# fjarri-attic/pyfft

Measured on AMD Instinct MI355X. Metric: batched_c2c_fft_gflops_5NlogN_1d_n2^20, higher is better.
Workload: dtype f32

## Files before the change

include/mifft.h:

```cpp
#ifndef MIFFT_H
#define MIFFT_H

#include <stddef.h>
#include <stdint.h>

#ifdef __cplusplus
extern "C" {
#endif

#define MIFFT_ABI_VERSION 6

#define MIFFT_E_INVALID      (-1)
#define MIFFT_E_UNSUPPORTED  (-2)
#define MIFFT_E_NODEVICE     (-3)

#define MIFFT_F32 0
#define MIFFT_F64 1

#define MIFFT_INTERLEAVED 0
#define MIFFT_SPLIT       1

#define MIFFT_FLAG_SRC_INTERLEAVED 1
#define MIFFT_FLAG_DST_INTERLEAVED 2
#define MIFFT_FLAG_STREAM_SRC 4
// ... 27 lines not shown
    int32_t tw_shift;
    int32_t src;
    int32_t dst;
    int32_t flags;
} mifft_pass;

typedef struct mifft_device_props {
    char    name[256];
    char    gcn_arch[64];
    int32_t compute_units;
    int32_t wavefront_size;
    int32_t max_threads_per_block;
    int32_t max_grid_x;
    int64_t lds_bytes_per_block;
    int64_t total_mem_bytes;
    int32_t clock_khz;
    int32_t l2_bytes;
    int64_t llc_bytes;
    int32_t num_xcc;
    int32_t reserved0;
} mifft_device_props;

int         mifft_abi_version(void);
const char *mifft_last_error(void);
#define MIFFT_DEBUG_NO_ND2 0
#define MIFFT_DEBUG_NO_WAVE 2
#define MIFFT_DEBUG_FORCE_WAVE 3
#define MIFFT_DEBUG_ALT_ROWS 5
#define MIFFT_DEBUG_PAIR 6
#define MIFFT_DEBUG_STORE 7
#define MIFFT_DEBUG_ROWS_ND 8
#define MIFFT_DEBUG_NARROW_TILES 9
#define MIFFT_DEBUG_NO_ROWFIRST 10
#define MIFFT_DEBUG_KEYS 12
int mifft_debug_set(int32_t key, int32_t value);
int mifft_debug_set_default(int32_t key, int32_t value);
int mifft_debug_get(int32_t key);

int mifft_device_count(int *count);
int mifft_set_device(int device);
int mifft_get_device(int *device);
int mifft_device_props_get(int device, mifft_device_props *props);
int mifft_malloc(void **ptr, size_t nbytes);
int mifft_free(void *ptr);
int mifft_memset(void *ptr, int value, size_t nbytes, mifft_stream_t stream);
int mifft_memcpy_h2d(void *dst, const void *src, size_t nbytes, mifft_stream_t stream);
int mifft_memcpy_d2h(void *dst, const void *src, size_t nbytes, mifft_stream_t stream);
int mifft_memcpy_d2d(void *dst, const void *src, size_t nbytes, mifft_stream_t stream);
int mifft_host_alloc(void **ptr, size_t nbytes);
int mifft_host_free(void *ptr);
int mifft_memcpy_d2h_async(void *dst, const void *src, size_t nbytes, mifft_stream_t stream);
int mifft_stream_create(mifft_stream_t *stream);
int mifft_stream_destroy(mifft_stream_t stream);
int mifft_stream_sync(mifft_stream_t stream);
int mifft_device_sync(void);
typedef void *mifft_graph_t;
int mifft_stream_is_capturing(mifft_stream_t stream, int32_t *capturing);
int mifft_stream_begin_capture(mifft_stream_t stream);
int mifft_stream_end_capture(mifft_stream_t stream, mifft_graph_t *graph);
int mifft_graph_launch(mifft_graph_t graph, mifft_stream_t stream);
int mifft_graph_destroy(mifft_graph_t graph);
int mifft_event_create(mifft_event_t *event);
int mifft_event_destroy(mifft_event_t event);
int mifft_event_record(mifft_event_t event, mifft_stream_t stream);
int mifft_event_sync(mifft_event_t event);
int mifft_event_query(mifft_event_t event);
int mifft_stream_wait_event(mifft_stream_t stream, mifft_event_t event);
int mifft_event_elapsed_ms(float *ms, mifft_event_t start, mifft_event_t stop);


// ... 163 lines not shown
```

pyfft_amd/_debug.py:

```python
import os


def forced_strategy():
    return os.environ.get("PYFFT_AMD_STRATEGY", "auto")


def pipeline_chunk_bytes(default):
    return (int(os.environ.get("PYFFT_AMD_PIPE_MB", "0")) << 20) or default


def no_nd_generic():
    return bool(os.environ.get("PYFFT_AMD_NO_ND_GENERIC"))


def pipeline_streams(default):
    return int(os.environ.get("PYFFT_AMD_PIPE_STREAMS", "0")) or default


def slab_bytes(default):
    return (int(os.environ.get("PYFFT_AMD_SLAB_MB", "0")) << 20) or default


def no_slabs():
    return bool(os.environ.get("PYFFT_AMD_NO_SLABS"))
# ... 40 lines not shown

def no_fusedp_alt():
    return bool(os.environ.get("PYFFT_AMD_NO_FUSEDP_ALT"))


def no_tiled_kernel():
    return bool(os.environ.get("PYFFT_AMD_NO_TILED"))


def no_mixed_nd():
    return bool(os.environ.get("PYFFT_AMD_NO_MIXED_ND"))


def fused3_lag_ring(lag, ring):
    v = os.environ.get("PYFFT_AMD_FUSED3")
    if v:
        lag, ring = (int(t) for t in v.split(","))
    return lag, ring


def apply_native_switches(native):
    for env, key in (("MIFFT_NO_ND2", native.DEBUG_NO_ND2), ("MIFFT_NO_WAVE", native.DEBUG_NO_WAVE),
                     ("MIFFT_FORCE_WAVE", native.DEBUG_FORCE_WAVE)):
        if os.environ.get(env):
            native.lib.mifft_debug_set_default(key, 1)
    if os.environ.get("MIFFT_STORE"):
        native.lib.mifft_debug_set_default(native.DEBUG_STORE, int(os.environ["MIFFT_STORE"]))
    if os.environ.get("MIFFT_ROWS_ND"):
        native.lib.mifft_debug_set_default(native.DEBUG_ROWS_ND, int(os.environ["MIFFT_ROWS_ND"]))
    if os.environ.get("MIFFT_NARROW_TILES"):
        native.lib.mifft_debug_set_default(native.DEBUG_NARROW_TILES, int(os.environ["MIFFT_NARROW_TILES"]))
    if os.environ.get("MIFFT_PAIR"):
        native.lib.mifft_debug_set_default(native.DEBUG_PAIR, int(os.environ["MIFFT_PAIR"]))
    if os.environ.get("PYFFT_AMD_NO_SPLIT_ROWFIRST"):
        native.lib.mifft_debug_set_default(native.DEBUG_NO_ROWFIRST, 1)
```

pyfft_amd/_native.py:

```python

import ctypes
import os

_HERE = os.path.dirname(os.path.abspath(__file__))
LIB_PATH = os.path.join(_HERE, "libmifft.so")

ABI_VERSION = 6
MIFFT_MIXED_MAX_STAGES = 12

E_INVALID = -1
E_UNSUPPORTED = -2
E_NODEVICE = -3

F32, F64 = 0, 1
INTERLEAVED, SPLIT = 0, 1
VARIANT_INTERLEAVED_ONLY = 2
VARIANT_SPLIT_ONLY = 3
VARIANT_OUT_OF_PLACE_ONLY = 4
VARIANT_OUT_OF_PLACE_ANY_SIZE = 5
VARIANT_SPLIT_OUT_OF_PLACE = 6
VARIANT_SPLIT_OUT_OF_PLACE_ANY_SIZE = 7
PASS_COL, PASS_ROW, PASS_ND = 0, 1, 2
FLAG_SRC_INTERLEAVED, FLAG_DST_INTERLEAVED = 1, 2
FLAG_STREAM_SRC, FLAG_STREAM_DST = 4, 8
FLAG_WRITE_THROUGH = 32
FLAG_PAIR_WITH_NEXT = 16
HALF_KERNEL_TILE, HALF_KERNEL_ROW, HALF_KERNEL_ND2, HALF_KERNEL_ND = 1, 2, 3, 4
ND_KERNEL_WAVE, ND_KERNEL_ND2Z, ND_KERNEL_ND2, ND_KERNEL_ND2ZP, ND_KERNEL_ND2P, ND_KERNEL_ND2T, ND_KERNEL_ND = 1, 2, 3, 4, 5, 6, 7
FUSED2_COUNTER_STRIDE = 64


def fused2_counter_bytes(outer):
    return FUSED2_COUNTER_STRIDE * 4 * (9 + 2 * int(outer))


DEBUG_NO_ND2, DEBUG_NO_WAVE, DEBUG_FORCE_WAVE, DEBUG_ALT_ROWS, DEBUG_PAIR, DEBUG_STORE = 0, 2, 3, 5, 6, 7
DEBUG_ROWS_ND = 8
DEBUG_NARROW_TILES = 9
DEBUG_NO_ROWFIRST = 10
DEBUG_KEYS = 12


class MifftPass(ctypes.Structure):
    _fields_ = [
        ("kind", ctypes.c_int32),
        ("precision", ctypes.c_int32),
        ("layout", ctypes.c_int32),
        ("inverse", ctypes.c_int32),
        ("L", ctypes.c_int32),
        ("variant", ctypes.c_int32),
        ("M", ctypes.c_int64),
        ("S", ctypes.c_int64),
        ("outer", ctypes.c_int64),
        ("outer_stride_in", ctypes.c_int64),
        ("outer_stride_out", ctypes.c_int64),
        ("scale", ctypes.c_double),
        ("tw_L", ctypes.c_void_p),
        ("tw_lo", ctypes.c_void_p),
        ("tw_hi", ctypes.c_void_p),
        ("tw_shift", ctypes.c_int32),
        ("src", ctypes.c_int32),
        ("dst", ctypes.c_int32),
        ("flags", ctypes.c_int32),
    ]


class MifftCopy(ctypes.Structure):
    _fields_ = [
        ("precision", ctypes.c_int32),
        ("ndim", ctypes.c_int32),
        ("dims", ctypes.c_int64 * 6),
        ("src_stride", ctypes.c_int64 * 6),
        ("dst_stride", ctypes.c_int64 * 6),
# ... 62 lines not shown

class MifftRealPost(ctypes.Structure):
    _fields_ = [
        ("precision", ctypes.c_int32),
        ("inverse", ctypes.c_int32),
        ("nx", ctypes.c_int32),
        ("ny", ctypes.c_int32),
        ("nz", ctypes.c_int32),
        ("reserved", ctypes.c_int32),
        ("outer", ctypes.c_int64),
        ("stride_in", ctypes.c_int64),
        ("stride_out", ctypes.c_int64),
        ("in_", ctypes.c_void_p),
        ("out", ctypes.c_void_p),
        ("tw", ctypes.c_void_p),
        ("scale", ctypes.c_double),
    ]


_vp = ctypes.c_void_p
_vpp = ctypes.POINTER(ctypes.c_void_p)
_i32 = ctypes.c_int32
_sz = ctypes.c_size_t
_pass_p = ctypes.POINTER(MifftPass)
_sync_p = ctypes.POINTER(MifftFusedSync)
_buf3 = ctypes.c_void_p * 3

PROTOTYPES = {
    "mifft_abi_version": (ctypes.c_int, []),
    "mifft_last_error": (ctypes.c_char_p, []),
    "mifft_debug_set": (ctypes.c_int, [_i32, _i32]),
    "mifft_debug_set_default": (ctypes.c_int, [_i32, _i32]),
    "mifft_debug_get": (ctypes.c_int, [_i32]),
    "mifft_device_count": (ctypes.c_int, [ctypes.POINTER(ctypes.c_int)]),
    "mifft_set_device": (ctypes.c_int, [ctypes.c_int]),
    "mifft_get_device": (ctypes.c_int, [ctypes.POINTER(ctypes.c_int)]),
    "mifft_device_props_get": (ctypes.c_int, [ctypes.c_int, ctypes.POINTER(MifftDeviceProps)]),
    "mifft_malloc": (ctypes.c_int, [_vpp, _sz]),
    "mifft_free": (ctypes.c_int, [_vp]),
    "mifft_memset": (ctypes.c_int, [_vp, ctypes.c_int, _sz, _vp]),
    "mifft_memcpy_h2d": (ctypes.c_int, [_vp, _vp, _sz, _vp]),
    "mifft_memcpy_d2h": (ctypes.c_int, [_vp, _vp, _sz, _vp]),
    "mifft_memcpy_d2d": (ctypes.c_int, [_vp, _vp, _sz, _vp]),
    "mifft_host_alloc": (ctypes.c_int, [_vpp, _sz]),
    "mifft_host_free": (ctypes.c_int, [_vp]),
    "mifft_memcpy_d2h_async": (ctypes.c_int, [_vp, _vp, _sz, _vp]),
    "mifft_stream_create": (ctypes.c_int, [_vpp]),
    "mifft_stream_destroy": (ctypes.c_int, [_vp]),
    "mifft_stream_sync": (ctypes.c_int, [_vp]),
    "mifft_device_sync": (ctypes.c_int, []),
    "mifft_stream_is_capturing": (ctypes.c_int, [_vp, ctypes.POINTER(ctypes.c_int32)]),
    "mifft_stream_begin_capture": (ctypes.c_int, [_vp]),
    "mifft_stream_end_capture": (ctypes.c_int, [_vp, _vpp]),
    "mifft_graph_launch": (ctypes.c_int, [_vp, _vp]),
    "mifft_graph_destroy": (ctypes.c_int, [_vp]),
    "mifft_event_create": (ctypes.c_int, [_vpp]),
    "mifft_event_destroy": (ctypes.c_int, [_vp]),
    "mifft_event_record": (ctypes.c_int, [_vp, _vp]),
    "mifft_event_sync": (ctypes.c_int, [_vp]),
    "mifft_event_query": (ctypes.c_int, [_vp]),
    "mifft_stream_wait_event": (ctypes.c_int, [_vp, _vp]),
    "mifft_event_elapsed_ms": (ctypes.c_int, [ctypes.POINTER(ctypes.c_float), _vp, _vp]),
    "mifft_nd_max_points_for": (ctypes.c_int, [_i32]),
    "mifft_nd_shape_supported": (ctypes.c_int, [_i32, _i32, _i32, _i32, _i32]),
    "mifft_pass_supported": (ctypes.c_int, [_i32, _i32, _i32, _i32]),
    "mifft_launch_pass": (ctypes.c_int, [_pass_p, _vp, _vp, _vp, _vp, _vp]),
# ... 94 lines not shown
```

pyfft_amd/csrc/fft_col2.hpp:

```cpp
#pragma once
#include "fft_tile.hpp"

namespace mifft {

template <int A, int E, typename T> __device__ __forceinline__ cplx<T> mul_w16A(cplx<T> v) {
    if constexpr (A == 4)
        return mul_w64<E, T>(v);
    else
        return mul_w32<E, T>(v);
}

template <typename T> struct ColStageTw {
    cplx<T> s1, s2, s3, s4, s5, s6, s7, s8;
    __device__ __forceinline__ void init(const cplx<T>* twL, int i0, int step = 1) {
        load(twL, i0, step);
        finish();
    }
    __device__ __forceinline__ void load(const cplx<T>* twL, int i0, int step = 1) {
        s1 = twL[step * i0]; s2 = twL[2 * step * i0]; s4 = twL[4 * step * i0]; s8 = twL[8 * step * i0];
    }
    __device__ __forceinline__ void finish() {
        s3 = cmul<T>(s1, s2); s5 = cmul<T>(s4, s1); s6 = cmul<T>(s4, s2); s7 = cmul<T>(s4, s3);
    }
    template <int k> __device__ __forceinline__ cplx<T> get() const {
        if constexpr (k == 1) return s1;
        else if constexpr (k == 2) return s2;
        else if constexpr (k == 3) return s3;
        else if constexpr (k == 4) return s4;
        else if constexpr (k == 5) return s5;
        else if constexpr (k == 6) return s6;
        else if constexpr (k == 7) return s7;
        else if constexpr (k == 8) return s8;
        else if constexpr (k == 9) return cmul<T>(s8, s1);
        else if constexpr (k == 10) return cmul<T>(s8, s2);
        else if constexpr (k == 11) return cmul<T>(s8, s3);
        else if constexpr (k == 12) return cmul<T>(s8, s4);
        else if constexpr (k == 13) return cmul<T>(s8, s5);
        else if constexpr (k == 14) return cmul<T>(s8, s6);
        else return cmul<T>(s8, s7);
    }
};

template <int A, bool TR, int ESZ = 8> struct Col2Lds {
    static constexpr int PITCH = TR ? 17 : 16;
    static constexpr int BUF = 16 * 16 * PITCH;
    static constexpr bool DOUBLE = A > 2 && ESZ <= 8;
    static constexpr bool HALF = ESZ > 8;
    static constexpr int ELEMS = HALF ? (BUF + 1) / 2 : (DOUBLE ? 2 : 1) * BUF;
};

struct TileNoHook {
    __device__ __forceinline__ void operator()() const {}
};

template <typename T, int A, bool TR, bool TW, bool SPLIT, bool WT = false, bool NTIN = false, bool NTOUT = false,
          bool SPLIT_OUT = SPLIT, bool WIDE = false, typename LdsPtr = cplx<T>*, typename Hook = TileNoHook>
__device__ __forceinline__ void col2_tile(const TileArgs& a, const long long o_in, const long long o_out,
                                          const long long rem0, LdsPtr lds, Hook hook = Hook(), const int tid_in = -1) {
    constexpr int L = A * 256;
    constexpr int PPT = A * 16;
    constexpr int PITCH = Col2Lds<A, TR, sizeof(cplx<T>)>::PITCH;
    constexpr int BUF = Col2Lds<A, TR, sizeof(cplx<T>)>::BUF;
    constexpr bool kDoubleBuf = Col2Lds<A, TR, sizeof(cplx<T>)>::DOUBLE;
    constexpr bool kHalf = Col2Lds<A, TR, sizeof(cplx<T>)>::HALF;

    int tid = tid_in >= 0 ? tid_in : (int)threadIdx.x;
    asm volatile("" : "+v"(tid));
    const int cg = WIDE ? (tid & 31) : (tid & 15), b0 = WIDE ? (tid >> 5) : (tid >> 4);
    const int c = cg & 15;
    if constexpr (WIDE) lds = lds + (cg >> 4) * Col2Lds<A, TR, sizeof(cplx<T>)>::ELEMS;
    int logMS = a.logMS, logS = a.logS;
    asm volatile("" : "+s"(logMS), "+s"(logS));
    const cplx<T>* twL = reinterpret_cast<const cplx<T>*>(a.tw_L);
    const T csign = a.inverse ? (T)-1 : (T)1;

    cplx<T> v[PPT];
    {
        const long long ubase = o_in * a.ostride_in + rem0;
        const unsigned voff = (((unsigned)b0 << logMS) + (unsigned)cg);
        if constexpr (!SPLIT) {
            const char* src = reinterpret_cast<const char*>(reinterpret_cast<const cplx<T>*>(a.in0) + ubase);
            const unsigned vb = voff * (unsigned)sizeof(cplx<T>);
            static_for<PPT>([&](auto kk) {
                constexpr int k = kk, ia = k >> 4, b1 = k & 15;
                const char* p = src + (((long long)(b1 * 16 * A + ia * 16) << logMS) * (long long)sizeof(cplx<T>));
                if constexpr (NTIN)
                    v[k] = __builtin_nontemporal_load(reinterpret_cast<const cplx<T>*>(p + vb));
                else
                    v[k] = *reinterpret_cast<const cplx<T>*>(p + vb);
            });
        } else {
            const char* sre = reinterpret_cast<const char*>(reinterpret_cast<const T*>(a.in0) + ubase);
            const char* sim = reinterpret_cast<const char*>(reinterpret_cast<const T*>(a.in1) + ubase);
            const unsigned vb = voff * (unsigned)sizeof(T);
            static_for<PPT>([&](auto kk) {
                constexpr int k = kk, ia = k >> 4, b1 = k & 15;
                const long long off = ((long long)(b1 * 16 * A + ia * 16) << logMS) * (long long)sizeof(T);
                if constexpr (NTIN) {
                    v[k].x = __builtin_nontemporal_load(reinterpret_cast<const T*>(sre + off + vb));
                    v[k].y = __builtin_nontemporal_load(reinterpret_cast<const T*>(sim + off + vb));
                } else {
                    v[k].x = *reinterpret_cast<const T*>(sre + off + vb);
                    v[k].y = *reinterpret_cast<const T*>(sim + off + vb);
                }
            });
        }
    }
    const cplx<T> s1 = twL[b0], s2 = twL[2 * b0], s4 = twL[4 * b0], s8 = twL[8 * b0];
    cplx<T> twA[A > 1 ? A - 1 : 1];
    if constexpr (A > 1) {
        static_for<A - 1>([&](auto qq) {
            constexpr int qa = qq + 1;
            twA[qq] = twL[16 * b0 * qa];
        });
    }
    __builtin_amdgcn_sched_barrier(0);
    static_for<PPT>([&](auto kk) {
        constexpr int k = kk;
        v[k].y *= csign;
    });

    {
        const cplx<T> s3 = cmul<T>(s1, s2), s5 = cmul<T>(s4, s1), s6 = cmul<T>(s4, s2), s7 = cmul<T>(s4, s3);
        auto tw = [&](auto kk) -> cplx<T> {
            constexpr int k = kk;
            if constexpr (k == 1) return s1;
            else if constexpr (k == 2) return s2;
            else if constexpr (k == 3) return s3;
            else if constexpr (k == 4) return s4;
            else if constexpr (k == 5) return s5;
            else if constexpr (k == 6) return s6;
            else if constexpr (k == 7) return s7;
            else if constexpr (k == 8) return s8;
            else if constexpr (k == 9) return cmul<T>(s8, s1);
            else if constexpr (k == 10) return cmul<T>(s8, s2);
            else if constexpr (k == 11) return cmul<T>(s8, s3);
            else if constexpr (k == 12) return cmul<T>(s8, s4);
            else if constexpr (k == 13) return cmul<T>(s8, s5);
            else if constexpr (k == 14) return cmul<T>(s8, s6);
            else return cmul<T>(s8, s7);
        };
        static_for<A>([&](auto aa) {
            constexpr int ia = aa;
            Dft<16, T>::run(v + ia * 16);
            static_for<15>([&](auto q2) {
                constexpr int qb1 = q2 + 1;
                cplx<T> t = v[ia * 16 + qb1];
                if constexpr (ia > 0) t = mul_w16A<A, ia * qb1, T>(t);
                v[ia * 16 + qb1] = cmul<T>(t, tw(IC<qb1>{}));
            });
            __builtin_amdgcn_sched_barrier(0);
        });
    }
    if constexpr (A > 1) {
        static_for<16>([&](auto bb) {
            constexpr int qb1 = bb;
            cplx<T> t[A];
            static_for<A>([&](auto aa) {
                constexpr int ia = aa;
                t[ia] = v[ia * 16 + qb1];
            });
            Dft<A, T>::run(t);
            v[qb1] = t[0];
            static_for<A - 1>([&](auto qq) {
                constexpr int qa = qq + 1;
                v[qa * 16 + qb1] = cmul<T>(t[qa], twA[qq]);
            });
        });
    }
    __builtin_amdgcn_sched_barrier(0);
    hook();

    const int u = TR ? c : b0;
    const int c2 = TR ? b0 : c;
    const int c2g = WIDE ? ((cg & 16) + c2) : c2;
    const long long l0 = rem0 >> logS;
    const long long jp0 = rem0 & ((1ll << logS) - 1);
    const unsigned dl = (unsigned)(((rem0 + c2g) >> logS) - l0);
    const unsigned djp = (unsigned)(((rem0 + c2g) & ((1ll << logS) - 1)) - jp0);
    const unsigned l = (unsigned)l0 + dl;
    const T sx = (T)a.scale;
    const T sy = a.inverse ? -sx : sx;
    cplx<T> sxy;
    sxy.x = sx;
    sxy.y = sy;
    const cplx<T>* twlo = reinterpret_cast<const cplx<T>*>(a.tw_lo);
    const cplx<T>* twhi = reinterpret_cast<const cplx<T>*>(a.tw_hi);
    const int tw_shift = a.tw_shift;
    const unsigned lomask = (1u << tw_shift) - 1u;
    const long long oubase = TR ? (a.ostride_out * o_out + rem0 * L) : (a.ostride_out * o_out + ((l0 * L) << logS) + jp0);
    const unsigned ovoff = TR ? ((unsigned)c2g * L + (unsigned)u) : ((((unsigned)dl * L + (unsigned)u) << logS) + djp);

    cplx<T> nlo[TW ? 4 : 1], nhi[TW ? 4 : 1], sstep_lo, sstep_hi;
    auto look_ahead = [&](auto qq) {
        constexpr int qa = qq;
        if constexpr (TW) {
            static_for<4>([&](auto jj) {
                constexpr int j = jj;
                const unsigned e = l * (unsigned)(qa * 16 + u + 64 * A * j);
                nlo[j] = twlo[e & lomask];
                nhi[j] = twhi[e >> tw_shift];
            });
        }
    };
    if constexpr (TW) {
        const unsigned e = l * (16u * A);
        sstep_lo = twlo[e & lomask];
        sstep_hi = twhi[e >> tw_shift];
        look_ahead(IC<0>{});
        __builtin_amdgcn_sched_barrier(0);
    }

    static_for<A>([&](auto rr) {
        constexpr int qa = rr;
        LdsPtr buf = lds + (kDoubleBuf ? (qa & 1) * BUF : 0);
        if constexpr (!kDoubleBuf && qa > 0) __syncthreads();
        cplx<T> x[16];
        if constexpr (!kHalf) {
            static_for<16>([&](auto ss) {
                constexpr int qb1 = ss;
                if constexpr (TR)
                    buf[(b0 * 16 + c) * PITCH + qb1] = v[qa * 16 + qb1];
                else
                    buf[(b0 * 16 + qb1) * 16 + c] = v[qa * 16 + qb1];
// ... 24 lines not shown
                    constexpr int bi = bb;
                    T w;
                    if constexpr (TR)
                        w = sb[(bi * 16 + c2) * PITCH + u];
                    else
                        w = sb[(bi * 16 + u) * 16 + c2];
                    if constexpr (comp == 0) x[bi].x = w; else x[bi].y = w;
                });
            });
        }
        cplx<T> anchor[TW ? 4 : 1];
        cplx<T> sstep;
        if constexpr (TW) {
            static_for<4>([&](auto jj) { anchor[jj] = cmul<T>(nlo[jj], nhi[jj]); });
            sstep = cmul<T>(sstep_lo, sstep_hi);
            __builtin_amdgcn_sched_barrier(0);
            if constexpr (qa + 1 < A) {
                look_ahead(IC<qa + 1>{});
                __builtin_amdgcn_sched_barrier(0);
            }
        }
        Dft<16, T>::run(x);
        if constexpr (TW) {
            static_for<4>([&](auto jj) {
                constexpr int j = jj;
                cplx<T> cur = anchor[j];
                static_for<4>([&](auto ii) {
                    constexpr int qb0 = 4 * j + ii;
                    x[qb0] = cmul<T>(x[qb0], cur);
                    if constexpr (ii < 3) cur = cmul<T>(cur, sstep);
                });
            });
        }
        static_for<16>([&](auto qq) {
            constexpr int qb0 = qq;
            const long long gu = TR ? (oubase + qb0 * 16 * A + 16 * qa)
                                    : (oubase + ((long long)(qb0 * 16 * A + 16 * qa) << logS));
            const cplx<T> r = x[qb0] * sxy;
            if constexpr (!SPLIT_OUT) {
                char* p = reinterpret_cast<char*>(reinterpret_cast<cplx<T>*>(a.out0) + gu);
                if constexpr (WT) {
                    if constexpr (sizeof(cplx<T>) == 8)
                        __hip_atomic_store(reinterpret_cast<unsigned long long*>(p + ovoff * (unsigned)sizeof(cplx<T>)),
                                           __builtin_bit_cast(unsigned long long, r), __ATOMIC_RELAXED, __HIP_MEMORY_SCOPE_AGENT);
                    else
                        store_wt<T>(p, ovoff * (unsigned)sizeof(cplx<T>), r);
                } else if constexpr (NTOUT) {
                    __builtin_nontemporal_store(r, reinterpret_cast<cplx<T>*>(p + ovoff * (unsigned)sizeof(cplx<T>)));
                } else {
                    *reinterpret_cast<cplx<T>*>(p + ovoff * (unsigned)sizeof(cplx<T>)) = r;
                }
            } else {
                char* pr = reinterpret_cast<char*>(reinterpret_cast<T*>(a.out0) + gu);
                char* pi = reinterpret_cast<char*>(reinterpret_cast<T*>(a.out1) + gu);
                if constexpr (NTOUT) {
                    __builtin_nontemporal_store(r.x, reinterpret_cast<T*>(pr + ovoff * (unsigned)sizeof(T)));
                    __builtin_nontemporal_store(r.y, reinterpret_cast<T*>(pi + ovoff * (unsigned)sizeof(T)));
                } else {
                    *reinterpret_cast<T*>(pr + ovoff * (unsigned)sizeof(T)) = r.x;
                    *reinterpret_cast<T*>(pi + ovoff * (unsigned)sizeof(T)) = r.y;
                }
            }
        });
    });
}

template <typename T, int A, bool TR, bool TW, bool SPLIT, bool SPLIT_OUT = SPLIT>
__global__ void __launch_bounds__(256, 2) fft_col2_kernel(const TileArgs a) {
    __shared__ __attribute__((aligned(16))) cplx<T> lds[Col2Lds<A, TR, sizeof(cplx<T>)>::ELEMS];
    const long long col0 = (long long)blockIdx.x * 16;
    const long long o = col0 >> a.logMS;
    const long long rem0 = col0 & ((1ll << a.logMS) - 1);
    if constexpr (TR && !SPLIT) {
        if (a.nt & 4) col2_tile<T, A, TR, TW, SPLIT, true, false, false, SPLIT_OUT>(a, o, o, rem0, lds);
        else if (a.nt & 1) col2_tile<T, A, TR, TW, SPLIT, false, !SPLIT, false, SPLIT_OUT>(a, o, o, rem0, lds);
        else col2_tile<T, A, TR, TW, SPLIT, false, false, false, SPLIT_OUT>(a, o, o, rem0, lds);
    } else if constexpr (!TR && !SPLIT_OUT) {
        if (a.nt & 4) col2_tile<T, A, TR, TW, SPLIT, true, false, false, SPLIT_OUT>(a, o, o, rem0, lds);
        else if (a.nt & 2) col2_tile<T, A, TR, TW, SPLIT, false, false, !SPLIT_OUT, SPLIT_OUT>(a, o, o, rem0, lds);
        else col2_tile<T, A, TR, TW, SPLIT, false, false, false, SPLIT_OUT>(a, o, o, rem0, lds);
    } else {
        col2_tile<T, A, TR, TW, SPLIT, false, false, false, SPLIT_OUT>(a, o, o, rem0, lds);
    }
}

template <int A, bool TR, bool TW, bool SPLIT, bool SPLIT_OUT>
__global__ void __launch_bounds__(512, 2) fft_col2x_kernel(const TileArgs a) {
    using T = float;
    __shared__ __attribute__((aligned(16))) cplx<T> lds[2 * Col2Lds<A, TR, sizeof(cplx<T>)>::ELEMS];
    const long long col0 = (long long)blockIdx.x * 32;
    const long long o = col0 >> a.logMS;
    const long long rem0 = col0 & ((1ll << a.logMS) - 1);
    const int tid = threadIdx.x;
    if constexpr (TR) {
        if (a.nt & 4) col2_tile<T, A, TR, TW, SPLIT, true, false, false, SPLIT_OUT, true>(a, o, o, rem0, lds, TileNoHook(), tid);
        else if (a.nt & 1) col2_tile<T, A, TR, TW, SPLIT, false, true, false, SPLIT_OUT, true>(a, o, o, rem0, lds, TileNoHook(), tid);
// ... 9 lines not shown
```

pyfft_amd/csrc/fft_fused2.hpp:

```cpp
#pragma once
#include "fft_col2.hpp"
#include "fft_col2w.hpp"
#include "fft_col3.hpp"

namespace mifft {

constexpr unsigned kFusedCS = 64u;

struct FusedCtl {
    unsigned* counters;
    unsigned* counters_next;
    unsigned* err;
    unsigned lines;
    unsigned batch;
    unsigned lag;
    unsigned ring;
    unsigned tiles0;
    unsigned tiles1;
};

struct FusedArgs {
    TileArgs p0;
    TileArgs p1;
    FusedCtl c;
// ... 145 lines not shown
        const FusedItem it = fused_decode<PER0, PER1>(f, item, gsize, wdone, rdone);
        if (it.pass == 2u) {
            fused_flush(pend);
            continue;
        }
        if (it.pass == 0u) {
            if (it.dep != nullptr) fused_wait_ge<false>(it.dep, it.target, seen, err, pend);
            else fused_flush(pend);
            if constexpr (EARLY) tile0(it.t, it.slot, it.tile, hook);
            else tile0(it.t, it.slot, it.tile, TileNoHook());
            pend.ctr = wdone + kFusedCS * it.t;
        } else {
            fused_wait_ge<true>(it.dep, it.target, seen, err, pend);
            if constexpr (EARLY) tile1(it.slot, it.t, it.tile, hook);
            else tile1(it.slot, it.t, it.tile, TileNoHook());
            fused_signal_read(rdone + kFusedCS * it.t);
        }
    }
    fused_flush(pend);
}

template <unsigned PER0, unsigned PER1, bool EARLY, typename TILE0, typename TILE1>
__device__ __forceinline__ void fused_loop(const FusedCtl& f, unsigned* s_item, TILE0&& tile0, TILE1&& tile1) {
    if (f.counters_next != nullptr) {
        for (unsigned i = blockIdx.x * blockDim.x + threadIdx.x; i < f.lines; i += gridDim.x * blockDim.x) {
            f.counters_next[i * kFusedCS] = 0u;
            f.counters_next[i * kFusedCS + 1u] = 0u;
        }
    }
    FusedPending pend = {};
    fused_list<PER0, PER1, EARLY>(f, s_item, tile0, tile1, pend);
}

template <typename T, int A0, int A1, bool SPLIT, int NT>
__global__ void __launch_bounds__(256, 2) fft_fused2_kernel(const FusedArgs f) {
    constexpr int E0 = Col2Lds<A0, true, sizeof(cplx<T>)>::ELEMS, E1 = Col2Lds<A1, false, sizeof(cplx<T>)>::ELEMS;
    __shared__ __attribute__((aligned(16))) cplx<T> lds[E0 > E1 ? E0 : E1];
    __shared__ unsigned s_item;
    constexpr unsigned per0 = A0 > A1 ? 1u : (unsigned)(A1 / A0);
    constexpr unsigned per1 = A1 > A0 ? 1u : (unsigned)(A0 / A1);
    fused_loop<per0, per1, !SPLIT && sizeof(T) == 4>(
        f.c, &s_item,
        [&](unsigned t, unsigned slot, unsigned tile, auto hook) {
            col2_tile<T, A0, true, true, SPLIT, true, NT != 0, false, false>(f.p0, (long long)t, (long long)slot, (long long)tile * 16, lds, hook);
        },
        [&](unsigned slot, unsigned t, unsigned tile, auto hook) {
            col2_tile<T, A1, false, false, false, NT == 2, false, NT == 1, SPLIT>(f.p1, (long long)slot, (long long)t, (long long)tile * 16, lds, hook);
        });
}

template <int A0, int A1, bool TWOD, bool NT = false, bool SPLIT = true>
__global__ void __launch_bounds__(512, 2) fft_fused2s_kernel(const FusedArgs f) {
    constexpr int E0 = Col2Lds<A0, true, sizeof(cplx<float>)>::ELEMS, E1 = Col2Lds<A1, TWOD, sizeof(cplx<float>)>::ELEMS;
    constexpr int E = E0 > E1 ? E0 : E1;
    __shared__ __attribute__((aligned(16))) cplx<float> lds[2 * E];
    __shared__ unsigned s_item;
    constexpr unsigned per0 = A0 > A1 ? 1u : (unsigned)(A1 / A0);
    constexpr unsigned per1 = A1 > A0 ? 1u : (unsigned)(A0 / A1);
    fused_loop<per0, per1, false>(
        f.c, &s_item,
        [&](unsigned t, unsigned slot, unsigned item, auto hook) {
            int tid = threadIdx.x;
            asm volatile("" : "+v"(tid));
            col2_tile<float, A0, true, !TWOD, SPLIT, true, NT, false, false, true>(f.p0, (long long)t, (long long)slot, (long long)item * 32, lds, hook, tid);
        },
        [&](unsigned slot, unsigned t, unsigned item, auto hook) {
            int tid = threadIdx.x;
            asm volatile("" : "+v"(tid));
            col2_tile<float, A1, TWOD, false, false, false, false, NT, SPLIT, true>(f.p1, (long long)slot, (long long)t, (long long)item * 32, lds, hook, tid);
        });
}

template <int A0, int A1>
__global__ void __launch_bounds__(256, 2) fft_fused2w_kernel(const FusedArgs f) {
    constexpr int E0 = Col2wLds<true>::ELEMS, E1 = Col2wLds<false>::ELEMS;
    __shared__ __attribute__((aligned(16))) cplx<float> lds[E0 > E1 ? E0 : E1];
    __shared__ unsigned s_item;
    constexpr unsigned per0 = A0 > A1 ? 1u : (unsigned)(A1 / A0);
    constexpr unsigned per1 = A1 > A0 ? 1u : (unsigned)(A0 / A1);
    fused_loop<per0, per1, (A0 == 1)>(
// ... 96 lines not shown
```

pyfft_amd/csrc/fft_fused2_f32.hip:

```cpp
#include "../../include/mifft.h"
#include "mifft_internal.h"
#include "fft_fused2.hpp"

namespace {
template <int A0, int A1> int launch(const mifft::FusedArgs* f, int split, unsigned grid, hipStream_t s) {
    if constexpr (A0 < A1) {
        return -2;
    } else {
        const int store = mifft_debug_get(MIFFT_DEBUG_STORE);
        if (mifft_debug_get(MIFFT_DEBUG_NARROW_TILES) == 1 || store == 2 || store == 3) return -2;
        if (split) {
            hipLaunchKernelGGL((mifft::fft_fused2s_kernel<A0, A1, false, true>), dim3(grid), dim3(512), 0, s, *f);
        } else if constexpr (A0 == 4) {
            hipLaunchKernelGGL((mifft::fft_fused2_kernel<float, A0, A1, false, 1>), dim3(grid), dim3(256), 0, s, *f);
        } else {
            return -2;
        }
        return (int)hipGetLastError();
    }
}
}

extern "C" int mifft_fused2_f32_launch(int L0, int L1, const mifft::FusedArgs* f, int split, unsigned grid, hipStream_t s) {
    if (L0 == 2048 && L1 == 2048) {
        if (split) hipLaunchKernelGGL((mifft::fft_fused3_kernel<float, 4, 4, true, true>), dim3(grid), dim3(512), 0, s, *f);
        else hipLaunchKernelGGL((mifft::fft_fused3_kernel<float, 4, 4, false, true>), dim3(grid), dim3(512), 0, s, *f);
        return (int)hipGetLastError();
    }
    if (L0 == 2048 && L1 == 1024) {
        if (split) hipLaunchKernelGGL((mifft::fft_fused3_kernel<float, 4, 2, true, true>), dim3(grid), dim3(512), 0, s, *f);
        else hipLaunchKernelGGL((mifft::fft_fused3_kernel<float, 4, 2, false, true>), dim3(grid), dim3(512), 0, s, *f);
        return (int)hipGetLastError();
    }
    const int key = (L0 / 256) * 10 + (L1 / 256);
    switch (key) {
        case 11: return launch<1, 1>(f, split, grid, s);
        case 12: return launch<1, 2>(f, split, grid, s);
        case 14: return launch<1, 4>(f, split, grid, s);
        case 21: return launch<2, 1>(f, split, grid, s);
        case 22: return launch<2, 2>(f, split, grid, s);
        case 24: return launch<2, 4>(f, split, grid, s);
        case 41: return launch<4, 1>(f, split, grid, s);
        case 42: return launch<4, 2>(f, split, grid, s);
        case 44: return launch<4, 4>(f, split, grid, s);
    }
// ... 14 lines not shown
```

pyfft_amd/csrc/mifft_internal.h:

```cpp
#pragma once
#include <hip/hip_runtime.h>
#include "../../include/mifft.h"
#include "fft_tile.hpp"
#include "fft_fused2.hpp"
#include "fft_nd.hpp"
#include "fft_wave.hpp"
#include "fft_pair.hpp"
#include "fft_nd2t.hpp"
#include "fft_fusedp.hpp"

extern "C" {
int mifft_dispatch_col_f32(int L, int tr, int variant, const mifft::TileArgs* a, hipStream_t s, int query_only);
int mifft_dispatch_row_f32(int L, int variant, const mifft::TileArgs* a, hipStream_t s, int query_only);
int mifft_dispatch_col_f64(int L, int tr, int variant, const mifft::TileArgs* a, hipStream_t s, int query_only);
int mifft_dispatch_row_f64(int L, int variant, const mifft::TileArgs* a, hipStream_t s, int query_only);
int mifft_nd_max_points(int f64);
int mifft_nd_launch(int f64, long long n, const mifft::NdArgs* a, hipStream_t s);
int mifft_nd2_f32_supported(int x, int y, int z);
int mifft_nd2_f32_launch(int x, int y, int z, const mifft::TileArgs* a, hipStream_t s);
int mifft_nd2_f64_supported(int x, int y, int z);
int mifft_nd2_f64_launch(int x, int y, int z, const mifft::TileArgs* a, hipStream_t s);
int mifft_fused2_f32_launch(int L0, int L1, const mifft::FusedArgs* f, int split, unsigned grid, hipStream_t s);
int mifft_fused2dw_f32(int ny, int nx, const mifft::FusedArgs* f, unsigned grid, hipStream_t s, int query, unsigned* tiles0, unsigned* tiles1);
int mifft_fused2r_f32(int ny, int nx, const mifft::FusedArgs* f, unsigned grid, hipStream_t s, int query);
int mifft_fused2w_f32_launch(int L0, int L1, const mifft::FusedArgs* f, unsigned grid, hipStream_t s);
int mifft_fused2d_f32_launch(int ny, int nx, const mifft::FusedArgs* f, int split, unsigned grid, hipStream_t s);
int mifft_fused3d_f64_launch(int ny, int nx, const mifft::FusedArgs* f, int split, unsigned grid, hipStream_t s);
int mifft_fusedx_f64(int L0, int L1, const mifft::FusedArgs* f, unsigned grid, hipStream_t s, int query, unsigned* tiles0, unsigned* tiles1);
int mifft_fused3_f64_launch(int L0, int L1, const mifft::FusedArgs* f, int split, unsigned grid, hipStream_t s);
int mifft_aux_copy_launch(const struct mifft_copy* c, const void* s0, const void* s1, void* d0, void* d1, hipStream_t s);
int mifft_aux_mul_rows_launch(int f64, void* a, const void* b, long long rows, long long n, hipStream_t s);
int mifft_aux_mul_spectrum_launch(int f64, void* data, const void* spectrum, long long items, long long points, long long spectrum_pitch,
                                  int correlate, double scale, hipStream_t s);
int mifft_aux_mismatch_launch(const void* a, const void* b, unsigned long long words, unsigned long long* count, hipStream_t s);
int mifft_aux_zero_launch(void* p, unsigned long long nbytes, hipStream_t s);
int mifft_wave_supported(int f64, int N);
int mifft_wave_launch(int f64, int N, const mifft::WaveArgs* a, int max_blocks, hipStream_t s);
int mifft_wave_16x16_launch(const mifft::WaveArgs* a, int max_blocks, hipStream_t s);
int mifft_pair_f64(int kind, int k0, int k1, int k2, int split, const mifft::PairArgs* a, hipStream_t s, int query, int* width);
int mifft_pair_f32(int kind, int k0, int k1, int k2, int split, const mifft::PairArgs* a, hipStream_t s, int query, int* width);
int mifft_fusedp(int f64, int split, int x, int y, int z, const mifft::FusedPairArgs* f, unsigned grid, hipStream_t s, int query, int* r0,
                 unsigned* tiles0, unsigned* tiles1);
int mifft_fusedp_more(int f64, int split, int x, int y, int z, const mifft::FusedPairArgs* f, unsigned grid, hipStream_t s, int query, int* r0,
                      unsigned* tiles0, unsigned* tiles1);
int mifft_nd2t(int f64, int x, int y, int z, const mifft::TileArgs* a, const mifft::TiledGeom* g, hipStream_t s, int query);
int mifft_nd2t_split_in(int f64, int x, int y, int z, const mifft::TileArgs* a, const mifft::TiledGeom* g, hipStream_t s, int query);
int mifft_nd2t_split(int f64, int x, int y, int z, const mifft::TileArgs* a, const mifft::TiledGeom* g, hipStream_t s, int query);
int mifft_nd2p(int f64, int x, int y, int z, const mifft::TileArgs* a, hipStream_t s, int query);
int mifft_nd2zp(int f64, int x, int y, int z, const mifft::TileArgs* a, hipStream_t s, int query);
int mifft_mixed_supported_impl(int f64, int n);
int mifft_mixed_radices_impl(int n, int32_t* radix);
int mifft_mixed_launch(int f64, int n, long long rows, long long stride_in, long long stride_out, long long inner, const void* in,
                       void* out, const void* tw, int flags, double scale, hipStream_t s);
int mifft_mixed_long_split_impl(int f64, long long n, int* n1, int* n2);
int mifft_mixed_long_launch(int f64, int n1, int n2, long long batch, const void* in, void* mid, void* out, const void* tw1, const void* tw2,
// ... 52 lines not shown
```

pyfft_amd/csrc/mifft_runtime.cpp:

```cpp
#include <hip/hip_runtime.h>
#include <hsa/hsa.h>
#include <hsa/hsa_ext_amd.h>

#include <atomic>
#include <cstdarg>
#include <cstdio>
#include <cstring>
#include <cstdlib>
#include <initializer_list>

#include "../../include/mifft.h"
#include "mifft_internal.h"
#include "fft_conv_row.hpp"

namespace {

thread_local char g_err[512] = "";
std::atomic<int> g_debug_default[MIFFT_DEBUG_KEYS];
thread_local int t_debug_value[MIFFT_DEBUG_KEYS];
thread_local unsigned t_debug_mask = 0;
struct DebugSwitches {
    int operator[](int key) const {
        return ((t_debug_mask >> key) & 1u) ? t_debug_value[key] : g_debug_default[key].load(std::memory_order_relaxed);
    }
};
const DebugSwitches g_debug;

int set_err(int code, const char* fmt, ...) {
    va_list ap;
    va_start(ap, fmt);
    vsnprintf(g_err, sizeof(g_err), fmt, ap);
    va_end(ap);
    return code;
}

int hip_check(hipError_t e, const char* what) {
    if (e == hipSuccess) return 0;
    return set_err((int)e, "%s: %s (%d)", what, hipGetErrorString(e), (int)e);
}

int launched(int rc) {
    if (rc == -1) return set_err(MIFFT_E_INVALID, "grid too large");
    return hip_check((hipError_t)rc, "kernel launch");
}

bool is_pow2(long long v) { return v > 0 && (v & (v - 1)) == 0; }
bool bad_precision(int precision) { return precision != MIFFT_F32 && precision != MIFFT_F64; }
long long complex_bytes(int precision) { return precision == MIFFT_F64 ? 16 : 8; }
bool misaligned(uintptr_t mask, std::initializer_list<const void*> ptrs) {
    uintptr_t all = 0;
    for (const void* p : ptrs) all |= (uintptr_t)p;
    return (all & mask) != 0;
}
// ... 378 lines not shown
    c->batch = (unsigned)outer;
    c->lag = (unsigned)lag;
    c->ring = (unsigned)ring_slots;
    c->tiles0 = tiles0;
    c->tiles1 = tiles1;
    if (!sync->counters_next) {
        hipStreamCaptureStatus st = hipStreamCaptureStatusNone;
        if (hipStreamIsCapturing(stream, &st) == hipSuccess && st == hipStreamCaptureStatusActive) {
            const int rz = mifft_aux_zero_launch(sync->counters, MIFFT_FUSED2_COUNTER_BYTES(outer), stream);
            return hip_check((hipError_t)rz, "kernel launch");
        }
        return hip_check(hipMemsetAsync(sync->counters, 0, MIFFT_FUSED2_COUNTER_BYTES(outer), stream), "hipMemsetAsync");
    }
    return 0;
}

}

extern "C" {

int mifft_abi_version(void) { return MIFFT_ABI_VERSION; }
int mifft_debug_set(int32_t key, int32_t value) {
    if (!debug_key_ok(key)) return set_err(MIFFT_E_INVALID, "bad debug key %d", key);
    t_debug_value[key] = value;
    t_debug_mask |= 1u << key;
    return 0;
}
int mifft_debug_set_default(int32_t key, int32_t value) {
    if (!debug_key_ok(key)) return set_err(MIFFT_E_INVALID, "bad debug key %d", key);
    g_debug_default[key].store(value, std::memory_order_relaxed);
    return 0;
}
int mifft_debug_get(int32_t key) { return (key >= 0 && key < MIFFT_DEBUG_KEYS) ? g_debug[key] : 0; }
const char* mifft_last_error(void) { return g_err; }

int mifft_device_count(int* count) {
    if (!count) return set_err(MIFFT_E_INVALID, "null argument");
    hipError_t e = hipGetDeviceCount(count);
    if (e == hipErrorNoDevice) {
        *count = 0;
        (void)hipGetLastError();
        return 0;
    }
    return hip_check(e, "hipGetDeviceCount");
}
int mifft_set_device(int device) { return hip_check(hipSetDevice(device), "hipSetDevice"); }
int mifft_get_device(int* device) { return hip_check(hipGetDevice(device), "hipGetDevice"); }

int mifft_device_props_get(int device, mifft_device_props* props) {
    if (!props) return set_err(MIFFT_E_INVALID, "null argument");
    hipDeviceProp_t p;
    int rc = hip_check(hipGetDeviceProperties(&p, device), "hipGetDeviceProperties");
    if (rc) return rc;
    memset(props, 0, sizeof(*props));
    snprintf(props->name, sizeof(props->name), "%s", p.name);
    snprintf(props->gcn_arch, sizeof(props->gcn_arch), "%s", p.gcnArchName);
    props->compute_units = p.multiProcessorCount;
    props->wavefront_size = p.warpSize;
    props->max_threads_per_block = p.maxThreadsPerBlock;
    props->max_grid_x = p.maxGridSize[0];
    props->lds_bytes_per_block = (int64_t)p.sharedMemPerBlock;
    props->total_mem_bytes = (int64_t)p.totalGlobalMem;
    props->clock_khz = p.clockRate;
    props->l2_bytes = p.l2CacheSize;
    probe_memory_system(p, &props->llc_bytes, &props->num_xcc);
    return 0;
// ... 967 lines not shown
```

Before: 21950.

## Pair lanes with permlane32 swap for 128-bit loads/stores in fused 1024x1024 FFT

Adds a paired-lane mode to the column tile kernel for the fp32 4x4 fused two-pass FFT. Each thread loads and stores two adjacent complex values as one 16-byte vector, and the values are exchanged between the lower and upper 32-lane halves with permlane32_swap to restore the original data mapping. The aim is to halve the number of memory instructions and widen global accesses for the 2^20-point case. In exchange it adds cross-lane swap instructions, a remapped thread-to-element indexing, an alignment check that falls back to the old kernel, and a new debug switch. It is enabled by default.

```diff
diff --git a/include/mifft.h b/include/mifft.h
--- a/include/mifft.h
+++ b/include/mifft.h
@@ -83,10 +83,12 @@
 #define MIFFT_DEBUG_ROWS_ND 8
 #define MIFFT_DEBUG_NARROW_TILES 9
 #define MIFFT_DEBUG_NO_ROWFIRST 10
-#define MIFFT_DEBUG_KEYS 12
+#define MIFFT_DEBUG_PAIR_LANES 12
+#define MIFFT_DEBUG_KEYS 13
 int mifft_debug_set(int32_t key, int32_t value);
 int mifft_debug_set_default(int32_t key, int32_t value);
 int mifft_debug_get(int32_t key);
+int mifft_debug_last_pair_lanes_form(void);
 
 int mifft_device_count(int *count);
 int mifft_set_device(int device);
diff --git a/pyfft_amd/_debug.py b/pyfft_amd/_debug.py
--- a/pyfft_amd/_debug.py
+++ b/pyfft_amd/_debug.py
@@ -96,5 +96,7 @@
         native.lib.mifft_debug_set_default(native.DEBUG_NARROW_TILES, int(os.environ["MIFFT_NARROW_TILES"]))
     if os.environ.get("MIFFT_PAIR"):
         native.lib.mifft_debug_set_default(native.DEBUG_PAIR, int(os.environ["MIFFT_PAIR"]))
+    if os.environ.get("MIFFT_PAIR_LANES"):
+        native.lib.mifft_debug_set_default(native.DEBUG_PAIR_LANES, int(os.environ["MIFFT_PAIR_LANES"]))
     if os.environ.get("PYFFT_AMD_NO_SPLIT_ROWFIRST"):
         native.lib.mifft_debug_set_default(native.DEBUG_NO_ROWFIRST, 1)
diff --git a/pyfft_amd/_native.py b/pyfft_amd/_native.py
--- a/pyfft_amd/_native.py
+++ b/pyfft_amd/_native.py
@@ -38,7 +38,8 @@
 DEBUG_ROWS_ND = 8
 DEBUG_NARROW_TILES = 9
 DEBUG_NO_ROWFIRST = 10
-DEBUG_KEYS = 12
+DEBUG_PAIR_LANES = 12
+DEBUG_KEYS = 13
 
 
 class MifftPass(ctypes.Structure):
@@ -167,6 +168,7 @@
     "mifft_debug_set": (ctypes.c_int, [_i32, _i32]),
     "mifft_debug_set_default": (ctypes.c_int, [_i32, _i32]),
     "mifft_debug_get": (ctypes.c_int, [_i32]),
+    "mifft_debug_last_pair_lanes_form": (ctypes.c_int, []),
     "mifft_device_count": (ctypes.c_int, [ctypes.POINTER(ctypes.c_int)]),
     "mifft_set_device": (ctypes.c_int, [ctypes.c_int]),
     "mifft_get_device": (ctypes.c_int, [ctypes.POINTER(ctypes.c_int)]),
diff --git a/pyfft_amd/csrc/fft_col2.hpp b/pyfft_amd/csrc/fft_col2.hpp
--- a/pyfft_amd/csrc/fft_col2.hpp
+++ b/pyfft_amd/csrc/fft_col2.hpp
@@ -53,8 +53,18 @@
     __device__ __forceinline__ void operator()() const {}
 };
 
+__device__ __forceinline__ void pair_swap(cplx<float>& lo, cplx<float>& hi) {
+    const float lx = lo.x, ly = lo.y, hx = hi.x, hy = hi.y;
+    const auto rx = __builtin_amdgcn_permlane32_swap(__builtin_bit_cast(unsigned, lx), __builtin_bit_cast(unsigned, hx), false, false);
+    const auto ry = __builtin_amdgcn_permlane32_swap(__builtin_bit_cast(unsigned, ly), __builtin_bit_cast(unsigned, hy), false, false);
+    const unsigned ax = rx[0], bx = rx[1], ay = ry[0], by = ry[1];
+    lo.x = __builtin_bit_cast(float, ax); hi.x = __builtin_bit_cast(float, bx);
+    lo.y = __builtin_bit_cast(float, ay); hi.y = __builtin_bit_cast(float, by);
+}
+
 template <typename T, int A, bool TR, bool TW, bool SPLIT, bool WT = false, bool NTIN = false, bool NTOUT = false,
-          bool SPLIT_OUT = SPLIT, bool WIDE = false, typename LdsPtr = cplx<T>*, typename Hook = TileNoHook>
+          bool SPLIT_OUT = SPLIT, bool WIDE = false, bool PAIR_IN = false, bool PAIR_OUT = false, typename LdsPtr = cplx<T>*,
+          typename Hook = TileNoHook>
 __device__ __forceinline__ void col2_tile(const TileArgs& a, const long long o_in, const long long o_out,
                                           const long long rem0, LdsPtr lds, Hook hook = Hook(), const int tid_in = -1) {
     constexpr int L = A * 256;
@@ -63,10 +73,16 @@
     constexpr int BUF = Col2Lds<A, TR, sizeof(cplx<T>)>::BUF;
     constexpr bool kDoubleBuf = Col2Lds<A, TR, sizeof(cplx<T>)>::DOUBLE;
     constexpr bool kHalf = Col2Lds<A, TR, sizeof(cplx<T>)>::HALF;
+    static_assert(!(PAIR_IN || PAIR_OUT) || (sizeof(T) == 4 && !WIDE && !kHalf), "paired lanes: fp32 16-column tiles only");
+    static_assert(!PAIR_IN || !SPLIT, "PAIR_IN: interleaved input only");
+    static_assert(!PAIR_OUT || !SPLIT_OUT, "PAIR_OUT: interleaved output only");
+    typedef T vec4 __attribute__((ext_vector_type(4)));
 
     int tid = tid_in >= 0 ? tid_in : (int)threadIdx.x;
     asm volatile("" : "+v"(tid));
-    const int cg = WIDE ? (tid & 31) : (tid & 15), b0 = WIDE ? (tid >> 5) : (tid >> 4);
+    const int upper = (tid >> 5) & 1;
+    const int pair_i = ((tid & 7) << 1) | upper, pair_j = ((tid >> 6) << 2) | ((tid >> 3) & 3);
+    const int cg = PAIR_IN ? pair_i : WIDE ? (tid & 31) : (tid & 15), b0 = PAIR_IN ? pair_j : WIDE ? (tid >> 5) : (tid >> 4);
     const int c = cg & 15;
     if constexpr (WIDE) lds = lds + (cg >> 4) * Col2Lds<A, TR, sizeof(cplx<T>)>::ELEMS;
     int logMS = a.logMS, logS = a.logS;
@@ -78,7 +94,20 @@
     {
         const long long ubase = o_in * a.ostride_in + rem0;
         const unsigned voff = (((unsigned)b0 << logMS) + (unsigned)cg);
-        if constexpr (!SPLIT) {
+        if constexpr (PAIR_IN) {
+            const char* src = reinterpret_cast<const char*>(reinterpret_cast<const cplx<T>*>(a.in0) + ubase);
+            const unsigned vb = ((((unsigned)b0 + (upper ? 16u * A : 0u)) << logMS) + (unsigned)(cg & ~1)) * (unsigned)sizeof(cplx<T>);
+            static_for<PPT / 2>([&](auto mm) {
+                constexpr int k = 2 * mm, ia = k >> 4, b1 = k & 15;
+                const char* p = src + (((long long)(b1 * 16 * A + ia * 16) << logMS) * (long long)sizeof(cplx<T>));
+                vec4 w;
+                if constexpr (NTIN)
+                    w = __builtin_nontemporal_load(reinterpret_cast<const vec4*>(p + vb));
+                else
+                    w = *reinterpret_cast<const vec4*>(p + vb);
+                v[k].x = w.x; v[k].y = w.y; v[k + 1].x = w.z; v[k + 1].y = w.w;
+            });
+        } else if constexpr (!SPLIT) {
             const char* src = reinterpret_cast<const char*>(reinterpret_cast<const cplx<T>*>(a.in0) + ubase);
             const unsigned vb = voff * (unsigned)sizeof(cplx<T>);
             static_for<PPT>([&](auto kk) {
@@ -115,6 +144,9 @@
         });
     }
     __builtin_amdgcn_sched_barrier(0);
+    if constexpr (PAIR_IN) {
+        static_for<PPT / 2>([&](auto mm) { pair_swap(v[2 * mm], v[2 * mm + 1]); });
+    }
     static_for<PPT>([&](auto kk) {
         constexpr int k = kk;
         v[k].y *= csign;
@@ -171,14 +203,16 @@
     __builtin_amdgcn_sched_barrier(0);
     hook();
 
-    const int u = TR ? c : b0;
-    const int c2 = TR ? b0 : c;
+    const int u = PAIR_OUT ? (TR ? pair_i : pair_j) : TR ? c : b0;
+    const int c2 = PAIR_OUT ? (TR ? pair_j : pair_i) : TR ? b0 : c;
     const int c2g = WIDE ? ((cg & 16) + c2) : c2;
+    const int c2s = (PAIR_OUT && !TR) ? (c2g & ~1) : c2g;
+    const int us = (PAIR_OUT && TR) ? (u & ~1) : u;
     const long long l0 = rem0 >> logS;
     const long long jp0 = rem0 & ((1ll << logS) - 1);
-    const unsigned dl = (unsigned)(((rem0 + c2g) >> logS) - l0);
-    const unsigned djp = (unsigned)(((rem0 + c2g) & ((1ll << logS) - 1)) - jp0);
-    const unsigned l = (unsigned)l0 + dl;
+    const unsigned dl = (unsigned)(((rem0 + c2s) >> logS) - l0);
+    const unsigned djp = (unsigned)(((rem0 + c2s) & ((1ll << logS) - 1)) - jp0);
+    const unsigned l = PAIR_OUT ? (unsigned)((rem0 + c2g) >> logS) : (unsigned)l0 + dl;
     const T sx = (T)a.scale;
     const T sy = a.inverse ? -sx : sx;
     cplx<T> sxy;
@@ -189,7 +223,8 @@
     const int tw_shift = a.tw_shift;
     const unsigned lomask = (1u << tw_shift) - 1u;
     const long long oubase = TR ? (a.ostride_out * o_out + rem0 * L) : (a.ostride_out * o_out + ((l0 * L) << logS) + jp0);
-    const unsigned ovoff = TR ? ((unsigned)c2g * L + (unsigned)u) : ((((unsigned)dl * L + (unsigned)u) << logS) + djp);
+    const unsigned ovoff = (TR ? ((unsigned)c2g * L + (unsigned)us) : ((((unsigned)dl * L + (unsigned)us) << logS) + djp)) +
+                           ((PAIR_OUT && upper) ? (TR ? 16u * A : ((16u * A) << logS)) : 0u);
 
     cplx<T> nlo[TW ? 4 : 1], nhi[TW ? 4 : 1], sstep_lo, sstep_hi;
     auto look_ahead = [&](auto qq) {
@@ -280,6 +315,24 @@
                 });
             });
         }
+        if constexpr (PAIR_OUT) {
+            static_for<8>([&](auto hh) {
+                constexpr int qb0 = 2 * hh;
+                const long long gu = TR ? (oubase + qb0 * 16 * A + 16 * qa)
+                                        : (oubase + ((long long)(qb0 * 16 * A + 16 * qa) << logS));
+                cplx<T> r0 = x[qb0] * sxy, r1 = x[qb0 + 1] * sxy;
+                pair_swap(r0, r1);
+                vec4 w;
+                w.x = r0.x; w.y = r0.y; w.z = r1.x; w.w = r1.y;
+                char* p = reinterpret_cast<char*>(reinterpret_cast<cplx<T>*>(a.out0) + gu);
+                if constexpr (WT)
+                    store_b128_sc1(p, ovoff * (unsigned)sizeof(cplx<T>), __builtin_bit_cast(unsigned __attribute__((ext_vector_type(4))), w));
+                else if constexpr (NTOUT)
+                    __builtin_nontemporal_store(w, reinterpret_cast<vec4*>(p + ovoff * (unsigned)sizeof(cplx<T>)));
+                else
+                    *reinterpret_cast<vec4*>(p + ovoff * (unsigned)sizeof(cplx<T>)) = w;
+            });
+        } else {
         static_for<16>([&](auto qq) {
             constexpr int qb0 = qq;
             const long long gu = TR ? (oubase + qb0 * 16 * A + 16 * qa)
@@ -310,6 +363,7 @@
                 }
             }
         });
+        }
     });
 }
 
diff --git a/pyfft_amd/csrc/fft_fused2.hpp b/pyfft_amd/csrc/fft_fused2.hpp
--- a/pyfft_amd/csrc/fft_fused2.hpp
+++ b/pyfft_amd/csrc/fft_fused2.hpp
@@ -201,8 +201,10 @@
     fused_list<PER0, PER1, EARLY>(f, s_item, tile0, tile1, pend);
 }
 
-template <typename T, int A0, int A1, bool SPLIT, int NT>
+constexpr int kPairIn = 1, kPairOut = 2;
+template <typename T, int A0, int A1, bool SPLIT, int NT, int PAIR0 = 0, int PAIR1 = 0>
 __global__ void __launch_bounds__(256, 2) fft_fused2_kernel(const FusedArgs f) {
+    static_assert((PAIR0 | PAIR1) == 0 || (sizeof(T) == 4 && A0 == 4 && A1 == 4 && !SPLIT && NT == 1), "paired lanes: <float, 4, 4, false, 1> only");
     constexpr int E0 = Col2Lds<A0, true, sizeof(cplx<T>)>::ELEMS, E1 = Col2Lds<A1, false, sizeof(cplx<T>)>::ELEMS;
     __shared__ __attribute__((aligned(16))) cplx<T> lds[E0 > E1 ? E0 : E1];
     __shared__ unsigned s_item;
@@ -211,10 +213,12 @@
     fused_loop<per0, per1, !SPLIT && sizeof(T) == 4>(
         f.c, &s_item,
         [&](unsigned t, unsigned slot, unsigned tile, auto hook) {
-            col2_tile<T, A0, true, true, SPLIT, true, NT != 0, false, false>(f.p0, (long long)t, (long long)slot, (long long)tile * 16, lds, hook);
-        },
-        [&](unsigned slot, unsigned t, unsigned tile, auto hook) {
-            col2_tile<T, A1, false, false, false, NT == 2, false, NT == 1, SPLIT>(f.p1, (long long)slot, (long long)t, (long long)tile * 16, lds, hook);
+            col2_tile<T, A0, true, true, SPLIT, true, NT != 0, false, false, false, (PAIR0 & kPairIn) != 0, (PAIR0 & kPairOut) != 0>(
+                f.p0, (long long)t, (long long)slot, (long long)tile * 16, lds, hook);
+        },
+        [&](unsigned slot, unsigned t, unsigned tile, auto hook) {
+            col2_tile<T, A1, false, false, false, NT == 2, false, NT == 1, SPLIT, false, (PAIR1 & kPairIn) != 0, (PAIR1 & kPairOut) != 0>(
+                f.p1, (long long)slot, (long long)t, (long long)tile * 16, lds, hook);
         });
 }
 
diff --git a/pyfft_amd/csrc/fft_fused2_f32.hip b/pyfft_amd/csrc/fft_fused2_f32.hip
--- a/pyfft_amd/csrc/fft_fused2_f32.hip
+++ b/pyfft_amd/csrc/fft_fused2_f32.hip
@@ -3,6 +3,19 @@
 #include "fft_fused2.hpp"
 
 namespace {
+constexpr int kPairLanesDefault = 3;
+int launch_1024(const mifft::FusedArgs* f, unsigned grid, hipStream_t s) {
+    constexpr int kPairAll = mifft::kPairIn | mifft::kPairOut;
+    const int sw = mifft_debug_get(MIFFT_DEBUG_PAIR_LANES);
+    int form = sw == 0 ? kPairLanesDefault : sw - 1;
+    if (form != 0 && form != 3) return -2;
+    if ((((uintptr_t)f->p0.in0 | (uintptr_t)f->p1.out0) & 15) != 0) form = 0;
+    if (form == 3) hipLaunchKernelGGL((mifft::fft_fused2_kernel<float, 4, 4, false, 1, kPairAll, kPairAll>), dim3(grid), dim3(256), 0, s, *f);
+    else hipLaunchKernelGGL((mifft::fft_fused2_kernel<float, 4, 4, false, 1>), dim3(grid), dim3(256), 0, s, *f);
+    mifft_note_pair_lanes_form(form);
+    return (int)hipGetLastError();
+}
+
 template <int A0, int A1> int launch(const mifft::FusedArgs* f, int split, unsigned grid, hipStream_t s) {
     if constexpr (A0 < A1) {
         return -2;
@@ -11,6 +24,8 @@
         if (mifft_debug_get(MIFFT_DEBUG_NARROW_TILES) == 1 || store == 2 || store == 3) return -2;
         if (split) {
             hipLaunchKernelGGL((mifft::fft_fused2s_kernel<A0, A1, false, true>), dim3(grid), dim3(512), 0, s, *f);
+        } else if constexpr (A0 == 4 && A1 == 4) {
+            return launch_1024(f, grid, s);
         } else if constexpr (A0 == 4) {
             hipLaunchKernelGGL((mifft::fft_fused2_kernel<float, A0, A1, false, 1>), dim3(grid), dim3(256), 0, s, *f);
         } else {
diff --git a/pyfft_amd/csrc/mifft_internal.h b/pyfft_amd/csrc/mifft_internal.h
--- a/pyfft_amd/csrc/mifft_internal.h
+++ b/pyfft_amd/csrc/mifft_internal.h
@@ -21,6 +21,7 @@
 int mifft_nd2_f64_supported(int x, int y, int z);
 int mifft_nd2_f64_launch(int x, int y, int z, const mifft::TileArgs* a, hipStream_t s);
 int mifft_fused2_f32_launch(int L0, int L1, const mifft::FusedArgs* f, int split, unsigned grid, hipStream_t s);
+void mifft_note_pair_lanes_form(int form);
 int mifft_fused2dw_f32(int ny, int nx, const mifft::FusedArgs* f, unsigned grid, hipStream_t s, int query, unsigned* tiles0, unsigned* tiles1);
 int mifft_fused2r_f32(int ny, int nx, const mifft::FusedArgs* f, unsigned grid, hipStream_t s, int query);
 int mifft_fused2w_f32_launch(int L0, int L1, const mifft::FusedArgs* f, unsigned grid, hipStream_t s);
diff --git a/pyfft_amd/csrc/mifft_runtime.cpp b/pyfft_amd/csrc/mifft_runtime.cpp
--- a/pyfft_amd/csrc/mifft_runtime.cpp
+++ b/pyfft_amd/csrc/mifft_runtime.cpp
@@ -19,6 +19,7 @@
 std::atomic<int> g_debug_default[MIFFT_DEBUG_KEYS];
 thread_local int t_debug_value[MIFFT_DEBUG_KEYS];
 thread_local unsigned t_debug_mask = 0;
+thread_local int t_pair_lanes_form = -1;
 struct DebugSwitches {
     int operator[](int key) const {
         return ((t_debug_mask >> key) & 1u) ? t_debug_value[key] : g_debug_default[key].load(std::memory_order_relaxed);
@@ -463,6 +464,8 @@
     return 0;
 }
 int mifft_debug_get(int32_t key) { return (key >= 0 && key < MIFFT_DEBUG_KEYS) ? g_debug[key] : 0; }
+void mifft_note_pair_lanes_form(int form) { t_pair_lanes_form = form; }
+int mifft_debug_last_pair_lanes_form(void) { return t_pair_lanes_form; }
 const char* mifft_last_error(void) { return g_err; }
 
 int mifft_device_count(int* count) {
```

After: 22460 (median of 6 runs). 1.02x the previous value.
